# refresh-bio/colord

Measured on AMD Instinct MI355X. Metric: input Gbases/s + archive size vs ref, ONT 50 Gb at 1/2/4/8 MI355X, higher is better.
Workload: dtype u64

## Files before the change

colord_amd/_native.py:

```python
from __future__ import annotations
import ctypes as C
import os

os.environ.setdefault("GPU_MAX_HW_QUEUES", "32")
_HERE = os.path.dirname(os.path.abspath(__file__))
LIB_PATH = os.environ.get("COLORD_HIP_LIBRARY") or os.path.join(_HERE, "libcolord_hip.so")

CL_OK, CL_E_INVALID, CL_E_HIP, CL_E_CAPACITY, CL_E_NOMEM, CL_E_UNSUPPORTED, CL_E_MISMATCH = 0, -1, -2, -3, -4, -5, -6


class ColordHipError(RuntimeError):
    def __init__(self, status, msg):
        super().__init__(f"colord_hip error {status}: {msg}")
        self.status = status


class QualParams(C.Structure):
    _fields_ = [("mode", C.c_int32), ("source", C.c_int32), ("level", C.c_int32), ("n_fwd", C.c_uint32), ("fwd", C.c_uint32 * 8),
                ("n_rev", C.c_uint32), ("rev", C.c_uint32 * 8)]


class KmerStats(C.Structure):
    _fields_ = [("n_reads", C.c_uint64), ("tot_kmers", C.c_uint64), ("n_unique", C.c_uint64),
                ("n_unique_counted", C.c_uint64), ("total_count_filtered", C.c_uint64)]
# ... 128 lines not shown
    "cl_accepted_kmers": (C.c_int32, [_P, _P, _P, C.c_uint32, C.c_uint32, C.POINTER(_P)]),
    "cl_kmer_lists_free": (None, [_P]),
    "cl_kmer_lists_reads": (C.c_uint32, [_P]),
    "cl_kmer_lists_total": (C.c_uint64, [_P]),
    "cl_kmer_lists_offsets": (_P, [_P]),
    "cl_kmer_lists_kmers": (_P, [_P]),
    "cl_kmer_lists_ids": (_P, [_P]),
    "cl_kmer_lists_pos": (_P, [_P]),
    "cl_ref_accept": (C.c_int32, [C.c_uint32, C.c_uint32, C.c_uint32, C.c_double, _P]),
    "cl_index_build": (C.c_int32, [_P, _P, _P, _P, C.c_uint32, C.c_uint32, C.POINTER(_P)]),
    "cl_index_entries_of": (C.c_int32, [_P, _P, _P, C.c_uint32, _P, _P, C.c_uint64, C.POINTER(C.c_uint64), _P, C.POINTER(C.c_uint32)]),
    "cl_index_build_pairs": (C.c_int32, [_P, _P, _P, _P, C.c_uint64, _P, C.c_uint32, C.c_uint32, C.c_uint32, C.c_uint32, C.POINTER(_P)]),
    "cl_index_free": (None, [_P]),
    "cl_index_n_refs": (C.c_uint32, [_P]),
    "cl_index_entries": (C.c_uint64, [_P]),
    "cl_index_ref_rank": (_P, [_P]),
    "cl_candidates": (C.c_int32, [_P, _P, _P, C.c_uint32, _P, _P, _P]),
    "cl_candidates_common": (C.c_int32, [_P, _P, _P, C.c_uint32, _P, _P, _P, _P, C.c_uint64, C.POINTER(C.c_uint64)]),
    "cl_qual_coder_create": (C.c_int32, [_P, C.POINTER(QualParams), C.POINTER(_P)]),
    "cl_qual_coder_ctx": (_P, [_P]),
    "cl_qual_coder_free": (None, [_P]),
    "cl_qual_coder_set_domain_symbols": (C.c_int32, [_P, C.c_uint64]),
    "cl_qual_coder_domains": (C.c_int32, [_P, _P, C.c_uint64, C.POINTER(C.c_uint64)]),
    "cl_qual_coder_model": (C.c_int32, [_P, C.c_uint32, C.c_uint64, _P, C.c_uint32, C.POINTER(C.c_uint32)]),
    "cl_qual_coder_groups": (C.c_int32, [_P, C.POINTER(C.c_uint64)]),
    "cl_compressor_set_qual_domain_symbols": (C.c_int32, [_P, C.c_uint64]),
    "cl_compressor_qual_domains": (C.c_int32, [_P, _P, C.c_uint64, C.POINTER(C.c_uint64)]),
    "cl_qual_decode_domains": (C.c_int32, [_P, C.POINTER(QualParams), _P, _P, _P, C.c_uint64, _P, _P, C.c_uint32, _P, C.c_uint32, C.c_uint32, _P, _P, C.c_uint64, _P, C.c_uint64]),
    "cl_qual_encode": (C.c_int32, [_P, _P, _P, _P, _P, _P, _P, C.c_uint32, _P, C.c_uint64, _P, C.POINTER(C.c_uint64)]),
    "cl_anchor_candidates": (C.c_int32, [_P, _P, _P, _P, _P, C.c_uint32, C.c_uint32, C.c_double, C.c_double, C.c_double, C.c_uint32, C.POINTER(_P)]),
    "cl_anchor_candidates_hifi": (C.c_int32, [_P, _P, _P, _P, _P, C.c_uint32, C.c_uint32, C.c_double, C.c_double, C.c_double, C.c_uint32, C.c_uint32, C.c_uint32, _P, _P, C.POINTER(_P)]),
    "cl_anchors_free": (None, [_P]),
    "cl_anchors_total": (C.c_uint64, [_P]),
    "cl_anchors_n_cands": (_P, [_P]),
    "cl_anchors_cands": (_P, [_P]),
    "cl_anchors_cand_offsets": (_P, [_P]),
    "cl_anchors_data": (_P, [_P]),
    "cl_encode_plain": (C.c_int32, [_P, _P, _P, C.c_uint64, _P, _P, C.POINTER(C.c_uint64)]),
    "cl_reads_select": (C.c_int32, [_P, _P, _P, C.POINTER(_P)]),
    "cl_reads_from_arena": (C.c_int32, [_P, _P, _P, _P, C.c_uint32, C.POINTER(_P)]),
    "cl_estimator_logs": (C.c_int32, [_P, _P, _P, C.c_uint64, _P]),
    "cl_es_flags": (C.c_int32, [_P, _P, _P, _P, _P, _P]),
    "cl_id_coder_create": (C.c_int32, [C.c_int32, C.POINTER(_P)]),
    "cl_id_coder_free": (None, [_P]),
    "cl_id_coder_error": (C.c_char_p, [_P]),
    "cl_id_encode_part": (C.c_int32, [_P, _P, _P, _P, C.c_uint32, _P, C.c_uint64, C.POINTER(C.c_uint64)]),
    "cl_compress_shard": (C.c_int32, [_P, C.POINTER(CompressParams), _P, _P, _P, _P, C.c_uint32, _P, C.c_uint32, _P, _P, _P, C.c_uint64, _P, _P, C.c_uint64, _P,
                                      C.POINTER(CompressInfo)]),
    "cl_candidates_at": (C.c_int32, [_P, _P, _P, _P, C.c_uint32, _P, _P, _P]),
    "cl_compressor_create": (C.c_int32, [_P, _P, C.POINTER(CompressParams), C.POINTER(QualParams), C.POINTER(Exchange), C.c_uint64, C.POINTER(_P)]),
    "cl_compressor_free": (None, [_P]),
    "cl_compressor_count_add": (C.c_int32, [_P, _P]),
    "cl_compressor_count_finish": (C.c_int32, [_P, C.POINTER(KmerStats)]),
    "cl_compressor_refs_add": (C.c_int32, [_P, _P]),
    "cl_compressor_refs_finish": (C.c_int32, [_P]),
    "cl_compressor_encode": (C.c_int32, [_P, _P, _P, _P, _P, C.c_uint32, _P, C.c_uint32, _P, C.c_uint64, _P, _P, C.c_uint64, _P, C.POINTER(CompressInfo)]),
    "cl_compressor_genome_add": (C.c_int32, [_P, _P]),
    "cl_compressor_pseudo_reads": (C.c_int32, [_P, _P]),
    "cl_genome_encode": (C.c_int32, [_P, _P, C.c_uint32, _P, C.c_uint64, C.POINTER(C.c_uint64)]),
    "cl_genome_decode": (C.c_int32, [_P, C.c_uint64, C.c_uint32, _P, C.c_uint64, _P, C.POINTER(C.c_uint64)]),
    "cl_genome_md5": (C.c_int32, [_P, _P, C.c_uint32, _P]),
    "cl_compressor_prepare": (C.c_int32, [_P, _P, _P, C.c_uint32]),
    "cl_compressor_prepare_parts": (C.c_int32, [_P, _P, _P, C.c_uint32, _P, C.c_uint32, _P, _P]),
    "cl_compressor_info": (C.c_int32, [_P, C.POINTER(KmerStats), C.POINTER(C.c_uint64), C.POINTER(C.c_uint64), C.POINTER(C.c_uint64), C.POINTER(C.c_uint32), C.POINTER(C.c_uint32)]),
    "cl_dna_decoder_create": (C.c_int32, [C.c_uint32, C.c_int32, C.c_uint32, C.c_uint32, C.c_int32, C.c_uint32, C.c_double, C.POINTER(_P)]),
    "cl_dna_decoder_free": (None, [_P]),
# ... 48 lines not shown
```

colord_amd/csrc/anchors.hip:

```cpp
#include "common.hpp"
#include "objects.hpp"
#include <algorithm>

struct cl_anchors {
	cl_ctx* ctx = nullptr;
	uint32_t n_reads = 0, c = 0;
	uint64_t n_anchors = 0;
	DevBuf<uint32_t> n_cands;
	DevBuf<uint32_t> cand;
	DevBuf<uint64_t> cand_off;
	DevBuf<uint32_t> anchors;
};

namespace {

struct Arena { const uint64_t* packed; const uint64_t* word_off; const uint32_t* lens; };

__device__ inline uint64_t mmer_at(const Arena& A, uint64_t wb, uint32_t p, uint32_t m)
{
	const uint64_t* w = A.packed + wb + (p >> 5);
	const uint32_t j = p & 31;
	const uint64_t hi = w[0], lo = w[1];
	const uint32_t s = 128 - 2 * (j + m);
	const uint64_t v = (s >= 64) ? (hi >> (s - 64)) : ((hi << (64 - s)) | (lo >> s));
	return v & ((1ULL << (2 * m)) - 1);
}
__device__ inline uint64_t mmer_of(uint64_t hi, uint64_t lo, uint32_t p, uint32_t m)
{
	const uint32_t s = 128 - 2 * ((p & 31) + m);
	const uint64_t v = (s >= 64) ? (hi >> (s - 64)) : ((hi << (64 - s)) | (lo >> s));
	return v & ((1ULL << (2 * m)) - 1);
}
__device__ inline uint64_t revcomp_m(uint64_t x, uint32_t m)
{
	x = ~x; x = __brevll(x);
	x = ((x >> 1) & 0x5555555555555555ULL) | ((x & 0x5555555555555555ULL) << 1);
	return x >> (64 - 2 * m);
}
__device__ inline uint64_t ref_mmer(const Arena& R, uint32_t id, bool rev, uint32_t q, uint32_t m)
{
	const uint32_t len = R.lens[id];
	const uint64_t wb = R.word_off[id];
	return rev ? revcomp_m(mmer_at(R, wb, len - m - q, m), m) : mmer_at(R, wb, q, m);
}
// ... 370 lines not shown
			};
			if (fill + tot > LSTAGE) flush();
			if (tot <= LSTAGE) { put(stage, (uint64_t)(fill + incl - cnt)); fill += tot; continue; }
			unsigned long long base = 0;
			if (lane == 0) base = atomicAdd(n_pairs, (unsigned long long)tot);
			base = ((unsigned long long)__shfl((int)(base >> 32), 0, 64) << 32) | (uint32_t)__shfl((int)(uint32_t)base, 0, 64);
			if (base + tot > cap) continue;
			put(pairs, (uint64_t)(base + incl - cnt));
		}
	}
	flush();
}
__global__ void k_task_pairs(const uint64_t* __restrict__ pairs, uint64_t n_pairs, Arena A, TaskCfg cfg, const uint32_t* __restrict__ n_distinct, uint32_t n_tasks,
                             uint64_t* __restrict__ pair_off, uint32_t* __restrict__ pair_cnt)
{
	const uint32_t t = blockIdx.x * blockDim.x + threadIdx.x;
	if (t > n_tasks) return;
	auto lower = [&](uint64_t task) -> uint64_t {
		const uint64_t key = task << (cfg.pe + cfg.pr);
		uint64_t lo = 0, hi = n_pairs;
		while (lo < hi) { const uint64_t mid = (lo + hi) >> 1; if (pairs[mid] < key) lo = mid + 1; else hi = mid; }
		return lo;
	};
	const uint64_t a = lower(t);
	pair_off[t] = a;
	if (t == n_tasks) return;
	uint32_t total = (uint32_t)(lower((uint64_t)t + 1) - a);
	const uint32_t rl = t / (2 * cfg.c); const uint32_t elen = A.lens[cfg.r0 + rl];
	const bool always = (double)n_distinct[rl] > cfg.frac_always * (double)elen;
	if (!always && (double)total > cfg.max_mult * (double)(elen + 1)) total = 0;
	pair_cnt[t] = total;
}

__device__ inline int lis_search(const int* __restrict__ tf, int size, int value)
{
	int low = 0;
	while (size > 0)
	{
		const int half = size / 2, other_half = size - half, probe = low + half, other_low = low + other_half;
		const int v = tf[probe];
		size = half;
		low = value > v ? other_low : low;
	}
	return low;
}
__global__ __launch_bounds__(64) void k_lis_anchors(Arena A, Arena R, TaskCfg cfg, const uint32_t* __restrict__ cand_refs, uint32_t n_tasks,
                                                   const uint64_t* __restrict__ pair_off, const uint32_t* __restrict__ pair_cnt, const uint64_t* __restrict__ pairs,
                                                   int* __restrict__ tf, int* __restrict__ ts, int* __restrict__ pred,
                                                   uint32_t* __restrict__ anch, uint32_t* __restrict__ t_nanch, uint32_t* __restrict__ t_tot, uint32_t dbg)
{
	__builtin_amdgcn_s_setprio(3);
	const uint32_t t = blockIdx.x * blockDim.x + threadIdx.x;
	if (t >= n_tasks) return;
	const uint64_t a = pair_off[t], b = a + pair_cnt[t];
	uint32_t n_anch = 0, tot = 0;
	if (b > a)
	{
		const uint32_t n = (uint32_t)(b - a);
		const uint64_t* P = pairs + a;
		int* F = tf + a; int* S = ts + a; int* PR = pred + a;
		const uint32_t pr_mask = (1u << cfg.pr) - 1, pe_mask = (1u << cfg.pe) - 1;
		auto ref_pos = [&](uint32_t i) -> int { return (int)(~(uint32_t)P[i] & pr_mask); };
		auto enc_pos = [&](uint32_t i) -> uint32_t { return (uint32_t)(P[i] >> cfg.pr) & pe_mask; };
		F[0] = ref_pos(0); S[0] = 0; PR[0] = -1;
		int out_len = 1;
		int last_f = F[0], last_s = 0;
		for (int i = 1; i < (int)n; ++i)
		{
			const int x = ref_pos((uint32_t)i);
			if (last_f < x)
			{
				F[out_len] = x; S[out_len] = i; PR[i] = last_s;
				++out_len; last_f = x; last_s = i;
				continue;
			}
			const int pos = lis_search(F, out_len, x);
			F[pos] = x; S[pos] = i;
			PR[i] = pos > 0 ? S[pos - 1] : -1;
			if (pos == out_len - 1) { last_f = x; last_s = i; }
		}
		if (dbg == 1) { t_nanch[t] = 0; t_tot[t] = 0; return; }
		int cur = S[out_len - 1];
		for (int i = out_len - 1; i >= 0; --i) { F[i] = cur; cur = PR[cur]; }
		if (dbg == 2) { t_nanch[t] = 0; t_tot[t] = 0; return; }
		const uint32_t rl = t / (2 * cfg.c), slot = (t / 2) % cfg.c; const bool rev = (t & 1) == 0;
		const uint32_t r = cfg.r0 + rl;
		const uint32_t id = cand_refs[(uint64_t)r * cfg.c + slot];
// ... 21 lines not shown
		int idx3 = idx_of(2);
		uint64_t pw2 = P[idx_of(1)];
		Raw w1 = words_of(P[idx_of(0)]);
		for (int i = 0; i < out_len; ++i)
		{
			const uint32_t pr = w1.pr, e_own = w1.e;
			const uint64_t mraw = m_from(w1.r0, w1.r1, w1.rp), mm = rev ? revcomp_m(mraw, cfg.m) : mraw, am = m_from(w1.a0, w1.a1, w1.e);
			w1 = words_of(pw2);
			pw2 = P[idx3];
			idx3 = idx_of(i + 3);
			uint32_t pe;
			for (;;)
			{
				pe = pe_at_ep;
				const bool hit = (pe == e_own ? am : mmer_at(A, ewb, pe, cfg.m)) == mm;
				uint32_t nxt = pe;
				do { ++ep; nxt = pe_ahead; pe_ahead = ep + 1 < n ? enc_pos(ep + 1) : 0xffffffffu; } while (ep < n && nxt == pe);
				pe_at_ep = nxt;
				if (hit || ep >= n) break;
			}
			if (run && prev_e == pe - 1 && prev_r == pr - 1) ++run;
			else
			{
				if (run) { out[3 * n_anch] = run + cfg.m - 1; out[3 * n_anch + 1] = start_e; out[3 * n_anch + 2] = start_r; tot += run + cfg.m - 1; ++n_anch; }
				run = 1; start_e = pe; start_r = pr;
			}
			prev_e = pe; prev_r = pr;
		}
		if (run) { out[3 * n_anch] = run + cfg.m - 1; out[3 * n_anch + 1] = start_e; out[3 * n_anch + 2] = start_r; tot += run + cfg.m - 1; ++n_anch; }
	}
	t_nanch[t] = n_anch; t_tot[t] = tot;
}

struct KmerArgs {
	const uint64_t* common; const uint64_t* common_off;
	uint64_t* sorted; uint32_t* tab;
	uint32_t* kanch;
	uint32_t* k_n; uint32_t* k_tot; uint8_t* k_use;
	uint64_t base;
	uint32_t k; ModTest mt;
};
__device__ inline uint32_t oriented_sym(const Arena& R, uint64_t wb, uint32_t len, bool rev, uint32_t pos)
{
	const uint32_t p = rev ? len - 1 - pos : pos;
	const uint32_t b = (uint32_t)(R.packed[wb + (p >> 5)] >> (62 - 2 * (p & 31))) & 3u;
	return rev ? 3u - b : b;
}
__device__ inline void kmer_occurrences(const Arena& A, uint64_t wb, uint32_t len, uint32_t k, const ModTest& mt, const uint64_t* sorted, uint32_t n, uint32_t* cntF, uint32_t* posF, uint32_t* cntR, uint32_t* posR)
{
	for (uint32_t i = 0; i < n; ++i) { cntF[i] = cntR[i] = 0; posF[i] = posR[i] = 0; }
	if (len < k) return;
	const uint64_t mask = (1ULL << (2 * k)) - 1; uint64_t f = 0, r = 0;
	for (uint32_t p = 0; p < len; ++p)
	{
		const uint64_t b = (A.packed[wb + (p >> 5)] >> (62 - 2 * (p & 31))) & 3u;
		f = ((f << 2) + b) & mask; r = (r >> 2) + ((3 - b) << (2 * (k - 1)));
		if (p + 1 < k) continue;
		const uint64_t can = f < r ? f : r;
		if (!mod_is_zero(hash_mm(can), mt)) continue;
		uint32_t lo = 0, hi = n;
		while (lo < hi) { const uint32_t mid = (lo + hi) >> 1; if (sorted[mid] < can) lo = mid + 1; else hi = mid; }
		if (lo >= n || sorted[lo] != can) continue;
		if (f == can) { ++cntF[lo]; posF[lo] = p + 1 - k; } else { ++cntR[lo]; posR[lo] = p + 1 - k; }
	}
}
__device__ inline uint32_t kmer_anchor_chain(const Arena& A, uint64_t ewb, uint32_t elen, const Arena& R, uint64_t rwb, uint32_t rlen, bool rev, uint32_t k,
// ... 199 lines not shown
	HIP_TRY(ctx, hipSetDevice(ctx->device));
	const uint32_t nr = reads->n_reads, m = anchor_len;
	cl_anchors* X = new cl_anchors(); X->ctx = ctx; X->n_reads = nr; X->c = c;
	std::unique_ptr<cl_anchors> guard(X);
	DEV_ALLOC(ctx, X->n_cands, nr); DEV_ALLOC(ctx, X->cand, (uint64_t)nr * c * 4); DEV_ALLOC(ctx, X->cand_off, (uint64_t)nr * c + 1);
	Arena A{ reads->packed.p, reads->word_off.p, reads->lens.p }, R{ refs->packed.p, refs->word_off.p, refs->lens.p };
	std::vector<uint32_t> h_len(nr);
	if (nr) HIP_TRY(ctx, hipMemcpy(h_len.data(), reads->lens.p, (uint64_t)nr * 4, hipMemcpyDeviceToHost));
	auto bits_for = [](uint64_t v) -> uint32_t { uint32_t b = 1; while ((1ull << b) <= v) ++b; return b; };
	uint32_t max_ref_len = 0;
	if (refs->n_reads)
	{
		std::vector<uint32_t> rl(refs->n_reads);
		HIP_TRY(ctx, hipMemcpy(rl.data(), refs->lens.p, (uint64_t)refs->n_reads * 4, hipMemcpyDeviceToHost));
		for (uint32_t l : rl) max_ref_len = std::max(max_ref_len, l);
	}
	const uint32_t pr_bits = bits_for(max_ref_len);
	const uint64_t BATCH_BASES = 1ull << 28;
	std::vector<DevBuf<uint32_t>> chunks; std::vector<uint64_t> chunk_n;
	uint64_t total_anchors = 0;
	double pairs_per_base = 0.5;
	struct TableBatch {
		uint32_t r0 = 0, r1 = 0, pe = 1; uint64_t acc = 0, nsum = 0;
		DevBuf<uint32_t> n_distinct, next, err; DevBuf<uint64_t> toff, noff; DevBuf<EncSlot> slots; DevBuf<uint2> bins;
		std::vector<uint2> h_work; DevBuf<uint2> work;
		struct SideSync { hipStream_t s = nullptr; ~SideSync() { if (s) (void)hipStreamSynchronize(s); } } sync;
	};
	HIP_TRY(ctx, cl_side_stream(ctx, ctx->side));
	constexpr uint32_t LDS_N_A = 12288, LDS_N_B = 24576, LDS_NT = 1024;
	uint32_t lds_max_n = 0;
	if (const char* e = getenv("COLORD_HIP_ANCHORS_LDS")) lds_max_n = atoi(e) <= 0 ? 0u : (uint32_t)atoi(e) <= LDS_N_A ? LDS_N_A : LDS_N_B;
	const uint32_t match_seg = getenv("COLORD_HIP_MATCH_SEG") ? (uint32_t)std::max(0, atoi(getenv("COLORD_HIP_MATCH_SEG"))) : 16384u;
	const uint32_t lds_dbg = getenv("COLORD_HIP_LDS_DBG") ? (uint32_t)atoi(getenv("COLORD_HIP_LDS_DBG")) : 0u;
	auto prepare = [&](uint32_t r0, std::unique_ptr<TableBatch>& out) -> cl_status {
		out = std::make_unique<TableBatch>();
		TableBatch& B = *out;
		uint32_t r1 = r0; uint64_t acc = 0;
		uint32_t mx = 0;
		while (r1 < nr && (r1 == r0 || acc + h_len[r1] <= BATCH_BASES))
		{
			const uint32_t pe = bits_for(std::max(mx, h_len[r1]));
			if (r1 > r0 && pe + pr_bits + bits_for((r1 - r0 + 1) * 2 * c) > 64) break;
			mx = std::max(mx, h_len[r1]); acc += h_len[r1]; ++r1;
		}
		B.r0 = r0; B.r1 = r1; B.acc = acc; B.pe = bits_for(mx);
		for (uint32_t r = r0; r < r1; ++r)
			for (uint32_t sg = 0, ns = match_segments(h_len[r] >= m ? h_len[r] - m + 1 : 0, match_seg); sg < ns; ++sg) B.h_work.push_back(make_uint2(r - r0, sg));
		if (B.pe + pr_bits + bits_for((r1 - r0) * 2 * c) > 64) return cl_fail(ctx, CL_E_UNSUPPORTED, "cl_anchor_candidates: a read and its candidates are too long for 64-bit match keys");
		const uint32_t nb = r1 - r0;
		const uint32_t table_x4 = 8;
		LaunchOn on(ctx, ctx->side);
		B.sync.s = ctx->side;
		DevBuf<uint32_t> tsize, nsize, err; DEV_ALLOC(ctx, tsize, nb); DEV_ALLOC(ctx, nsize, nb); DEV_ALLOC(ctx, err, 1); DEV_ALLOC(ctx, B.n_distinct, nb);
		HIP_TRY(ctx, hipMemsetAsync(err.p, 0, 4, ctx->side));
		LAUNCH(ctx, k_table_sizes, grid_for(nb, 256), 256, (const uint32_t*)reads->lens.p, (const uint8_t*)reads->has_n.p, d_cand_n, r0, r1, m, table_x4, lds_max_n, tsize.p, nsize.p, err.p);
		DEV_ALLOC(ctx, B.toff, (uint64_t)nb + 1); DEV_ALLOC(ctx, B.noff, (uint64_t)nb + 1);
		uint64_t tsum = 0;
		CL_TRY(dev_exclusive_scan_u64(ctx, tsize.p, B.toff.p, nb, &tsum));
		CL_TRY(dev_exclusive_scan_u64(ctx, nsize.p, B.noff.p, nb, &B.nsum));
		uint32_t herr = 0; HIP_TRY(ctx, hipMemcpyAsync(&herr, err.p, 4, hipMemcpyDeviceToHost, ctx->side)); HIP_TRY(ctx, hipStreamSynchronize(ctx->side));
		DEV_ALLOC(ctx, B.slots, tsum); DEV_ALLOC(ctx, B.next, B.nsum); DEV_ALLOC(ctx, B.bins, B.nsum); DEV_ALLOC(ctx, B.err, 1);
		DEV_ALLOC(ctx, B.work, B.h_work.size() + 1);
		if (!B.h_work.empty()) HIP_TRY(ctx, hipMemcpyAsync(B.work.p, B.h_work.data(), B.h_work.size() * sizeof(uint2), hipMemcpyHostToDevice, ctx->side));
		HIP_TRY(ctx, hipMemsetAsync(B.n_distinct.p, 0, (uint64_t)nb * 4, ctx->side));
		HIP_TRY(ctx, hipMemsetAsync(B.err.p, 0, 4, ctx->side));
		EncTable T{ B.slots.p, B.toff.p, B.next.p, B.noff.p };
// ... 24 lines not shown
			DEV_ALLOC(ctx, pairs, cap);
			HIP_TRY(ctx, hipMemsetAsync(d_np.p, 0, 32, ctx->stream));
			if (lds_max_n)
			{
				LAUNCH_NAMED(ctx, "k_match_lds<12288>", (k_match_lds<LDS_N_A, 2048, LDS_NT, 8>), nb, LDS_NT, A, R, cfg, 0u, (const uint8_t*)reads->has_n.p, d_cand_refs, d_cand_n, n_distinct.p, nb, d_np.p, cap, pairs.p, lds_dbg);
				if (lds_max_n > LDS_N_A)
					LAUNCH_NAMED(ctx, "k_match_lds<24576>", (k_match_lds<LDS_N_B, 4096, LDS_NT, 4>), nb, LDS_NT, A, R, cfg, LDS_N_A, (const uint8_t*)reads->has_n.p, d_cand_refs, d_cand_n, n_distinct.p, nb, d_np.p, cap, pairs.p, lds_dbg);
			}
			LAUNCHB(ctx, 0.0, k_match, (uint32_t)cur->h_work.size(), 256, A, R, T, cfg, d_cand_refs, d_cand_n, (const uint32_t*)n_distinct.p, (const uint2*)cur->work.p, (uint32_t)cur->h_work.size(), match_seg, d_np.p, cap, pairs.p);
			HIP_TRY(ctx, hipGetLastError());
			unsigned long long h_np2[2] = { 0, 0 };
			HIP_TRY(ctx, hipMemcpyAsync(h_np2, d_np.p, 16, hipMemcpyDeviceToHost, ctx->stream));
			if (r1 < nr && !nxt) CL_TRY(prepare(r1, nxt));
			HIP_TRY(ctx, hipStreamSynchronize(ctx->stream));
			const unsigned long long h_np = h_np2[0];
			n_pairs = h_np;
			if (ctx->timing && !ctx->pending_bytes.empty()) ctx->pending_bytes.back() = (double)h_np2[1] * 8.25 + (double)std::min<uint64_t>(h_np, cap) * 8.0;
			if (getenv("COLORD_HIP_ANCHOR_DEBUG")) fprintf(stderr, "[anchors] batch reads %u..%u bases %llu: pairs %llu cap %llu\n", r0, r1, (unsigned long long)acc, h_np, (unsigned long long)cap);
			if (n_pairs >= (1ull << 32)) return cl_fail(ctx, CL_E_UNSUPPORTED, "cl_anchor_candidates: batch produces >= 2^32 match pairs");
			if (n_pairs <= cap) break;
			cap = n_pairs;
		}
		if (acc) pairs_per_base = std::max(pairs_per_base, (double)n_pairs / (double)acc);
		DevBuf<int> tf, ts, pred; DEV_ALLOC(ctx, tf, n_pairs); DEV_ALLOC(ctx, ts, n_pairs); DEV_ALLOC(ctx, pred, n_pairs);
		DevBuf<uint32_t> anch; DEV_ALLOC(ctx, anch, 3 * n_pairs);
		DevBuf<uint32_t> t_nanch, t_tot; DEV_ALLOC(ctx, t_nanch, n_tasks); DEV_ALLOC(ctx, t_tot, n_tasks);
		if (n_pairs)
		{
			uint32_t tb = 1; while ((1ull << tb) < n_tasks) ++tb;
			CL_TRY(dev_sort_pairs(ctx, pairs.p, nullptr, n_pairs, 0, cfg.pe + cfg.pr + tb));
		}
		LAUNCH(ctx, k_task_pairs, grid_for((uint64_t)n_tasks + 1, 256), 256, (const uint64_t*)pairs.p, n_pairs, A, cfg, (const uint32_t*)n_distinct.p, n_tasks, pair_off.p, pair_cnt.p);
		LAUNCHB(ctx, n_pairs * 32.0, k_lis_anchors, grid_for(n_tasks, 64), 64, A, R, cfg, d_cand_refs, n_tasks, (const uint64_t*)pair_off.p, (const uint32_t*)pair_cnt.p, (const uint64_t*)pairs.p,
			tf.p, ts.p, pred.p, anch.p, t_nanch.p, t_tot.p, (uint32_t)(getenv("COLORD_HIP_LIS_DBG") ? atoi(getenv("COLORD_HIP_LIS_DBG")) : 0));
		HIP_TRY(ctx, hipGetLastError());
		const uint64_t n_slots = (uint64_t)nb * c;
		DevBuf<uint64_t> k_sorted; DevBuf<uint32_t> k_tab, kanch, k_n, k_tot; DevBuf<uint8_t> k_use;
		uint64_t common_base = 0;
		if (hifi)
		{
			uint64_t hb[2] = { 0, 0 };
			HIP_TRY(ctx, hipMemcpy(&hb[0], d_common_off + (uint64_t)r0 * c, 8, hipMemcpyDeviceToHost));
			HIP_TRY(ctx, hipMemcpy(&hb[1], d_common_off + (uint64_t)r1 * c, 8, hipMemcpyDeviceToHost));
			common_base = hb[0];
			const uint64_t nk = hb[1] - hb[0];
			DEV_ALLOC(ctx, k_sorted, nk + 1); DEV_ALLOC(ctx, k_tab, 8 * nk + 8); DEV_ALLOC(ctx, kanch, 6 * nk + 6);
			DEV_ALLOC(ctx, k_n, 2 * n_slots); DEV_ALLOC(ctx, k_tot, 2 * n_slots); DEV_ALLOC(ctx, k_use, n_slots);
			KmerArgs ka{ d_common, d_common_off, k_sorted.p, k_tab.p, kanch.p, k_n.p, k_tot.p, k_use.p, common_base, kmer_len, make_modtest(modulo) };
			LAUNCH(ctx, k_kmer_anchors, grid_for(n_slots, 64), 64, A, R, cfg, d_cand_refs, d_cand_n, (const uint8_t*)reads->has_n.p, (const uint32_t*)n_distinct.p, ka);
			HIP_TRY(ctx, hipGetLastError());
		}
		DevBuf<uint32_t> o_task, o_count; DEV_ALLOC(ctx, o_task, n_slots); DEV_ALLOC(ctx, o_count, n_slots);
		LAUNCH(ctx, k_select, grid_for(nb, 128), 128, cfg, d_cand_refs, d_cand_n, min_anchors, (const uint32_t*)t_nanch.p, (const uint32_t*)t_tot.p,
			(const uint8_t*)(hifi ? k_use.p : nullptr), (const uint32_t*)k_n.p, (const uint32_t*)k_tot.p,
			X->n_cands.p, X->cand.p, o_task.p, o_count.p);
		DevBuf<uint64_t> slot_off; DEV_ALLOC(ctx, slot_off, n_slots + 1);
		uint64_t n_here = 0;
		CL_TRY(dev_exclusive_scan_u64(ctx, o_count.p, slot_off.p, n_slots, &n_here));
		DevBuf<uint32_t> chunk; DEV_ALLOC(ctx, chunk, 3 * n_here);
		LAUNCH(ctx, k_copy_fix, grid_for(n_slots, 128), 128, (const uint32_t*)o_task.p, (const uint64_t*)slot_off.p, n_slots, (const uint64_t*)pair_off.p,
			(const uint32_t*)anch.p, (uint64_t)0, chunk.p, cfg, (const uint32_t*)kanch.p, d_common_off, common_base);
		HIP_TRY(ctx, hipMemcpyAsync(X->cand_off.p + (uint64_t)r0 * c, slot_off.p, n_slots * 8, hipMemcpyDeviceToDevice, ctx->stream));
		if (total_anchors) LAUNCH(ctx, k_add_u64, grid_for(n_slots, 256), 256, X->cand_off.p + (uint64_t)r0 * c, n_slots, total_anchors);
		HIP_TRY(ctx, hipGetLastError());
		HIP_TRY(ctx, hipStreamSynchronize(ctx->stream));
		chunks.push_back(std::move(chunk)); chunk_n.push_back(n_here);
		total_anchors += n_here;
		cur = std::move(nxt);
	}
	X->n_anchors = total_anchors;
	DEV_ALLOC(ctx, X->anchors, 3 * total_anchors);
	uint64_t o = 0;
	for (size_t i = 0; i < chunks.size(); ++i)
	{
		if (chunk_n[i]) HIP_TRY(ctx, hipMemcpyAsync(X->anchors.p + 3 * o, chunks[i].p, chunk_n[i] * 12, hipMemcpyDeviceToDevice, ctx->stream));
		o += chunk_n[i];
	}
	HIP_TRY(ctx, hipMemcpyAsync(X->cand_off.p + (uint64_t)nr * c, &total_anchors, 8, hipMemcpyHostToDevice, ctx->stream));
	HIP_TRY(ctx, hipStreamSynchronize(ctx->stream));
	cl_timing_collect(ctx);
	*out = guard.release();
	return CL_OK;
}
extern "C" void cl_anchors_free(cl_anchors* a) { delete a; }
extern "C" uint64_t cl_anchors_total(const cl_anchors* a) { return a->n_anchors; }
extern "C" const uint32_t* cl_anchors_n_cands(const cl_anchors* a) { return a->n_cands.p; }
extern "C" const uint32_t* cl_anchors_cands(const cl_anchors* a) { return a->cand.p; }
extern "C" const uint64_t* cl_anchors_cand_offsets(const cl_anchors* a) { return a->cand_off.p; }
extern "C" const uint32_t* cl_anchors_data(const cl_anchors* a) { return a->anchors.p; }
```

colord_amd/device.py:

```python
from __future__ import annotations
import ctypes as C
import numpy as np
import torch
from . import _native as N


def _check(ctx, st):
    if ctx is not None and getattr(ctx, "timing", False):
        for n, (ms, k, b, cells) in ctx.kernel_times().items():
            a = ctx.acc.setdefault(n, [0.0, 0, 0.0, 0.0])
            a[0] += ms
            a[1] += k
            a[2] += b
            a[3] += cells
    if st != N.CL_OK:
        msg = N.load().cl_last_error(ctx.h).decode() if ctx is not None and ctx.h else ""
        raise N.ColordHipError(st, msg)


def _view(ptr, n, dtype, device):
    out = torch.empty(int(n), dtype=dtype, device=device)
    if n:
        torch.cuda.synchronize(device)
        rc = _hip().hipMemcpy(C.c_void_p(out.data_ptr()), C.c_void_p(ptr), C.c_size_t(int(n) * out.element_size()), 3)
# ... 757 lines not shown
    def __init__(self, ctx, h, max_alt_refs):
        super().__init__(ctx, h)
        self.max_alt_refs = max_alt_refs

    def encode(self, refs: "Reads", es: torch.Tensor, es_off: torch.Tensor, es_ntuples: torch.Tensor, part_bounds):
        ctx = self.ctx
        pb = np.ascontiguousarray(part_bounds, dtype=np.uint32)
        n_parts = len(pb) - 1
        n_reads = es_off.numel() - 1
        sizes = np.zeros(max(n_parts, 1), np.uint64)
        cap = max(4096, int(es.numel() * 0.6) + 64 * n_parts)
        out = torch.empty(cap, dtype=torch.uint8, device=ctx.device)
        n = C.c_uint64(0)
        st = ctx.lib.cl_dna_encode(ctx.h, self.h, refs.h, es.data_ptr(), es_off.data_ptr(), es_ntuples.data_ptr(), n_reads,
                                   pb.ctypes.data, n_parts, out.data_ptr(), cap, sizes.ctypes.data, C.byref(n))
        _check(ctx, st)
        return out[:n.value], [int(x) for x in sizes[:n_parts]]

    def model(self, family: int, context: int) -> np.ndarray:
        out = np.zeros(257, np.uint32)
        _check(self.ctx, self.ctx.lib.cl_dna_coder_model(self.h, family, context, out.ctypes.data))
        return out[:(self.N_SYM[family] or self.max_alt_refs) + 1].copy()


class Anchors(_Obj):
    _free = "cl_anchors_free"

    def __init__(self, ctx, h, n_reads, c):
        super().__init__(ctx, h)
        self.n_reads, self.c = n_reads, c

    @property
    def total(self): return self.ctx.lib.cl_anchors_total(self.h)
    def n_cands(self): return self._arr("cl_anchors_n_cands", self.n_reads, torch.int32)
    def cands(self): return self._arr("cl_anchors_cands", self.n_reads * self.c * 4, torch.int32).view(self.n_reads, self.c, 4)
    def cand_offsets(self): return self._arr("cl_anchors_cand_offsets", self.n_reads * self.c + 1, torch.int64)
    def data(self): return self._arr("cl_anchors_data", self.total * 3, torch.int32).view(-1, 3)
```

include/colord_hip.h:

```cpp
#ifndef COLORD_HIP_H
#define COLORD_HIP_H
#include <stdint.h>
#include <stddef.h>

#ifdef __cplusplus
extern "C" {
#endif

typedef int32_t cl_status;
enum {
	CL_OK = 0,
	CL_E_INVALID = -1,
	CL_E_HIP = -2,
	CL_E_CAPACITY = -3,
	CL_E_NOMEM = -4,
	CL_E_UNSUPPORTED = -5,
	CL_E_MISMATCH = -6
};

typedef struct cl_ctx cl_ctx;
typedef struct cl_reads cl_reads;
typedef struct cl_kmer_set cl_kmer_set;
typedef struct cl_kmer_lists cl_kmer_lists;
typedef struct cl_index cl_index;
// ... 81 lines not shown

typedef struct cl_qual_coder cl_qual_coder;
typedef struct {
	int32_t mode;
	int32_t source;
	int32_t level;
	uint32_t n_fwd;
	uint32_t fwd[8];
	uint32_t n_rev;
	uint32_t rev[8];
} cl_qual_params;
cl_status cl_qual_coder_create(cl_ctx* ctx, const cl_qual_params* params, cl_qual_coder** out);
void cl_qual_coder_free(cl_qual_coder* q);
cl_ctx* cl_qual_coder_ctx(const cl_qual_coder* q);
cl_status cl_qual_encode(cl_ctx* ctx, cl_qual_coder* q, const cl_reads* reads, const uint8_t* d_quals, const uint64_t* d_qual_off,
                         const uint8_t* d_flags, const uint32_t* h_part_bounds, uint32_t n_parts,
                         uint8_t* d_out, uint64_t cap, uint64_t* h_part_sizes, uint64_t* n_out);

cl_status cl_qual_coder_set_domain_symbols(cl_qual_coder* q, uint64_t n);
cl_status cl_qual_coder_domains(const cl_qual_coder* q, uint64_t* h_first_part, uint64_t cap, uint64_t* n_out);
cl_status cl_qual_coder_model(const cl_qual_coder* q, uint32_t family, uint64_t context, uint32_t* out, uint32_t cap, uint32_t* n_out);
cl_status cl_qual_coder_groups(const cl_qual_coder* q, uint64_t* n_out);

typedef struct cl_anchors cl_anchors;
cl_status cl_anchor_candidates(cl_ctx* ctx, const cl_reads* reads, const cl_reads* refs, const uint32_t* d_cand_refs, const uint32_t* d_cand_n,
                               uint32_t c, uint32_t anchor_len, double frac_always, double frac_min, double max_matches_mult,
                               uint32_t min_anchors, cl_anchors** out);
cl_status cl_anchor_candidates_hifi(cl_ctx* ctx, const cl_reads* reads, const cl_reads* refs, const uint32_t* d_cand_refs, const uint32_t* d_cand_n,
                                    uint32_t c, uint32_t anchor_len, double frac_always, double frac_min, double max_matches_mult,
                                    uint32_t min_anchors, uint32_t kmer_len, uint32_t modulo, const uint64_t* d_common_off, const uint64_t* d_common,
                                    cl_anchors** out);
void cl_anchors_free(cl_anchors* a);
uint64_t cl_anchors_total(const cl_anchors* a);
const uint32_t* cl_anchors_n_cands(const cl_anchors* a);
const uint32_t* cl_anchors_cands(const cl_anchors* a);
const uint64_t* cl_anchors_cand_offsets(const cl_anchors* a);
const uint32_t* cl_anchors_data(const cl_anchors* a);

cl_status cl_encode_plain(cl_ctx* ctx, const cl_reads* reads, uint8_t* d_es, uint64_t cap, uint64_t* d_es_off,
                          uint32_t* d_es_ntuples, uint64_t* n_out);

cl_status cl_encode_reads(cl_ctx* ctx, const cl_reads* reads, const cl_reads* refs, const cl_anchors* anchors, uint32_t c, uint32_t anchor_len,
                          uint32_t min_part_alt, uint32_t max_rec, double cost_mult, const uint32_t* h_pack_bounds, uint32_t n_packs,
                          uint8_t* d_es, uint64_t cap, uint64_t* d_es_off, uint32_t* d_es_ntuples, uint64_t* n_out);

cl_status cl_estimator_logs(cl_ctx* ctx, const uint32_t* d_count, const uint32_t* d_total, uint64_t n, double* d_out);

cl_status cl_es_flags(cl_ctx* ctx, const cl_reads* reads, const uint8_t* d_es, const uint64_t* d_es_off, const uint64_t* d_base_off, uint8_t* d_flags);

cl_status cl_es_expand(cl_ctx* ctx, const cl_reads* refs, const uint8_t* d_es, const uint64_t* d_es_off, const uint32_t* d_es_ntuples, uint32_t n_reads,
                       uint8_t* d_codes, uint64_t cap, uint64_t* d_base_off, uint64_t* n_out);
cl_status cl_es_verify(cl_ctx* ctx, const cl_reads* reads, const cl_reads* refs, const uint8_t* d_es, const uint64_t* d_es_off, const uint32_t* d_es_ntuples,
                       uint64_t* n_bad, uint32_t* first_bad);

cl_status cl_digest_bases(cl_ctx* ctx, const cl_reads* reads, uint64_t first_read, cl_digest* acc);
cl_status cl_digest_quals(cl_ctx* ctx, const cl_qual_params* qparams, const cl_reads* reads, const uint8_t* d_quals, const uint64_t* d_qual_off,
                          uint64_t first_read, cl_digest* acc);
cl_status cl_digest_bases_host(const uint8_t* h_codes, const uint64_t* h_off, uint64_t n, uint64_t first_read, cl_digest* acc);
cl_status cl_digest_bytes_host(uint32_t kind, const uint8_t* h_bytes, const uint64_t* h_off, uint64_t n, uint64_t first_read, cl_digest* acc);
cl_status cl_digest_qual_values(cl_ctx* ctx, const cl_qual_params* qparams, const cl_reads* reads, const uint8_t* d_quals, const uint64_t* d_qual_off,
                                uint64_t first_read, cl_digest* acc);
cl_status cl_qual_values(cl_ctx* ctx, const cl_qual_params* qparams, const cl_reads* reads, const uint8_t* d_quals, const uint64_t* d_qual_off,
                         uint8_t* d_values, uint64_t cap);
cl_status cl_qual_values_host(const cl_qual_params* qparams, const uint8_t* h_quals, const uint64_t* h_off, uint64_t n, uint8_t* h_values);
cl_status cl_digest_qual_values_host(const uint8_t* h_ascii_quals, const uint64_t* h_off, uint64_t n, uint64_t first_read, cl_digest* acc);

// ... 154 lines not shown
```

Measured before the change: 2.927.

## Chain long anchor candidate lists with a whole wavefront instead of one lane

Tasks whose pair list has at least a threshold number of entries (default 64) are skipped by the per-lane LIS kernel. A new kernel then processes each such task with a full 64-lane wavefront: it extends runs with ballots, uses a wave-parallel binary search for the LIS, backtracks in parallel and emits anchors cooperatively. The aim is to remove load imbalance and serial latency from lanes stuck on long lists. It adds an extra kernel launch, atomic counters with a reduction kernel and a small device-to-host copy, and brings complex lane-cooperative logic that must match the serial output exactly.

```diff
diff --git a/colord_amd/_native.py b/colord_amd/_native.py
--- a/colord_amd/_native.py
+++ b/colord_amd/_native.py
@@ -184,6 +184,10 @@
     "cl_anchor_candidates_hifi": (C.c_int32, [_P, _P, _P, _P, _P, C.c_uint32, C.c_uint32, C.c_double, C.c_double, C.c_double, C.c_uint32, C.c_uint32, C.c_uint32, _P, _P, C.POINTER(_P)]),
     "cl_anchors_free": (None, [_P]),
     "cl_anchors_total": (C.c_uint64, [_P]),
+    "cl_anchors_wave_tasks": (C.c_uint64, [_P]),
+    "cl_anchors_wave_pairs": (C.c_uint64, [_P]),
+    "cl_anchors_lane_tasks": (C.c_uint64, [_P]),
+    "cl_anchors_lane_pairs": (C.c_uint64, [_P]),
     "cl_anchors_n_cands": (_P, [_P]),
     "cl_anchors_cands": (_P, [_P]),
     "cl_anchors_cand_offsets": (_P, [_P]),
diff --git a/colord_amd/csrc/anchors.hip b/colord_amd/csrc/anchors.hip
--- a/colord_amd/csrc/anchors.hip
+++ b/colord_amd/csrc/anchors.hip
@@ -10,6 +10,8 @@
 	DevBuf<uint32_t> cand;
 	DevBuf<uint64_t> cand_off;
 	DevBuf<uint32_t> anchors;
+	DevBuf<unsigned long long> lis_counts_d;
+	unsigned long long lis_counts[6] = { 0, 0, 0, 0, 0, 0 };
 };
 
 namespace {
@@ -446,6 +448,22 @@
 	pair_cnt[t] = total;
 }
 
+constexpr uint32_t LIS_COUNT_LINES = 1024;
+__device__ inline unsigned long long shfl_xor_u64(unsigned long long v, int d)
+{
+	return ((unsigned long long)(uint32_t)__shfl_xor((int)(v >> 32), d, 64) << 32) | (uint32_t)__shfl_xor((int)(uint32_t)v, d, 64);
+}
+__global__ __launch_bounds__(64) void k_lis_counts_sum(unsigned long long* __restrict__ counts)
+{
+	unsigned long long v[6] = { 0, 0, 0, 0, 0, 0 };
+	for (uint32_t l = threadIdx.x; l < LIS_COUNT_LINES; l += 64)
+		for (int k = 0; k < 6; ++k) { const unsigned long long x = counts[(size_t)l * 8 + k]; v[k] = k == 5 ? max(v[k], x) : v[k] + x; }
+	for (int d = 32; d; d >>= 1)
+		for (int k = 0; k < 6; ++k) { const unsigned long long x = shfl_xor_u64(v[k], d); v[k] = k == 5 ? max(v[k], x) : v[k] + x; }
+	__syncthreads();
+	if (threadIdx.x == 0) for (int k = 0; k < 6; ++k) counts[k] = v[k];
+}
+
 __device__ inline int lis_search(const int* __restrict__ tf, int size, int value)
 {
 	int low = 0;
@@ -461,12 +479,25 @@
 __global__ __launch_bounds__(64) void k_lis_anchors(Arena A, Arena R, TaskCfg cfg, const uint32_t* __restrict__ cand_refs, uint32_t n_tasks,
                                                    const uint64_t* __restrict__ pair_off, const uint32_t* __restrict__ pair_cnt, const uint64_t* __restrict__ pairs,
                                                    int* __restrict__ tf, int* __restrict__ ts, int* __restrict__ pred,
-                                                   uint32_t* __restrict__ anch, uint32_t* __restrict__ t_nanch, uint32_t* __restrict__ t_tot, uint32_t dbg)
+                                                   uint32_t* __restrict__ anch, uint32_t* __restrict__ t_nanch, uint32_t* __restrict__ t_tot,
+                                                   uint32_t wave_min, unsigned long long* __restrict__ counts, uint32_t dbg)
 {
 	__builtin_amdgcn_s_setprio(3);
 	const uint32_t t = blockIdx.x * blockDim.x + threadIdx.x;
-	if (t >= n_tasks) return;
-	const uint64_t a = pair_off[t], b = a + pair_cnt[t];
+	const uint32_t n_own = t < n_tasks ? pair_cnt[t] : 0;
+	const bool others = n_own && wave_min && n_own >= wave_min;
+	{
+		unsigned long long sum = others ? 0 : n_own; uint32_t mx = (uint32_t)sum;
+		for (int d = 32; d; d >>= 1) { sum += shfl_xor_u64(sum, d); mx = max(mx, (uint32_t)__shfl_xor((int)mx, d, 64)); }
+		const uint32_t tasks = (uint32_t)__popcll(__ballot(n_own && !others));
+		if ((threadIdx.x & 63) == 0 && tasks)
+		{
+			unsigned long long* cl = counts + (size_t)(blockIdx.x % LIS_COUNT_LINES) * 8;
+			atomicAdd(cl + 2, (unsigned long long)tasks); atomicAdd(cl + 3, sum); atomicMax(cl + 5, (unsigned long long)mx);
+		}
+	}
+	if (t >= n_tasks || others) return;
+	const uint64_t a = pair_off[t], b = a + n_own;
 	uint32_t n_anch = 0, tot = 0;
 	if (b > a)
 	{
@@ -554,6 +585,182 @@
 	t_nanch[t] = n_anch; t_tot[t] = tot;
 }
 
+__device__ inline void lis_wave_fence() { __builtin_amdgcn_fence(__ATOMIC_ACQ_REL, "workgroup"); }
+__device__ inline uint64_t shfl_u64(uint64_t v, uint32_t src)
+{
+	return ((uint64_t)(uint32_t)__shfl((int)(v >> 32), (int)src, 64) << 32) | (uint32_t)__shfl((int)(uint32_t)v, (int)src, 64);
+}
+__device__ inline uint32_t ones_from_bit0(uint64_t b) { return b == ~0ULL ? 64u : (uint32_t)__builtin_ctzll(~b); }
+__device__ inline int lis_search_wave(const int* F, int size, int value, uint32_t lane)
+{
+	int lo = 0;
+	while (size > 0)
+	{
+		const int piece = (size + 63) >> 6, end = lo + size;
+		const long long idx = (long long)lo + ((long long)lane + 1) * piece - 1;
+		const bool less = idx < end && F[idx] < value;
+		lo += __popcll(__ballot(less)) * piece;
+		size = min(piece - 1, end - lo);
+	}
+	return lo;
+}
+constexpr uint32_t LIS_WAVE_GAP = 8;
+constexpr uint32_t LIS_WAVE_BLOCK = 256;
+constexpr uint32_t LIS_WAVE_MIN_DEFAULT = 64;
+__global__ __launch_bounds__(LIS_WAVE_BLOCK) void k_lis_anchors_wave(Arena A, Arena R, TaskCfg cfg, const uint32_t* __restrict__ cand_refs, uint32_t n_tasks,
+                                                        const uint64_t* __restrict__ pair_off, const uint32_t* __restrict__ pair_cnt, const uint64_t* __restrict__ pairs,
+                                                        int* tf, int* ts, int* pred, uint32_t* __restrict__ anch, uint32_t* __restrict__ t_nanch, uint32_t* __restrict__ t_tot,
+                                                        uint32_t wave_min, unsigned long long* __restrict__ counts, uint32_t dbg)
+{
+	__builtin_amdgcn_s_setprio(3);
+	const uint32_t lane = threadIdx.x & 63;
+	const uint32_t t = __builtin_amdgcn_readfirstlane(blockIdx.x * (LIS_WAVE_BLOCK / 64) + (threadIdx.x >> 6));
+	if (t >= n_tasks) return;
+	const uint32_t n = pair_cnt[t];
+	if (n == 0 || n < wave_min) return;
+	const uint64_t a = pair_off[t];
+	const uint64_t* P = pairs + a;
+	int* F = tf + a; int* S = ts + a; int* PR = pred + a;
+	const uint32_t m = cfg.m, pr_mask = (1u << cfg.pr) - 1, pe_mask = (1u << cfg.pe) - 1;
+	auto ref_pos = [&](uint32_t i) -> int { return (int)(~(uint32_t)P[i] & pr_mask); };
+	auto enc_pos = [&](uint32_t i) -> uint32_t { return (uint32_t)(P[i] >> cfg.pr) & pe_mask; };
+	unsigned long long* cl = counts + (size_t)(blockIdx.x % LIS_COUNT_LINES) * 8;
+	if (lane == 0) { atomicAdd(cl, 1ULL); atomicAdd(cl + 1, (unsigned long long)n); atomicMax(cl + 5, (unsigned long long)n); }
+	uint32_t n_slow = 0;
+	int out_len = 0, last_f = -1, last_s = -1;
+	for (uint32_t i0 = 0; i0 < n; i0 += 64)
+	{
+		const uint32_t cnt = min(64u, n - i0);
+		const int x = lane < cnt ? ref_pos(i0 + lane) : 0;
+		const int xp = __shfl_up(x, 1, 64);
+		uint32_t k0 = 0;
+		while (k0 < cnt)
+		{
+			const bool ext = lane >= k0 && lane < cnt && x > (lane == k0 ? last_f : xp);
+			const uint32_t r = ones_from_bit0(__ballot(ext) >> k0);
+			if (r)
+			{
+				if (lane >= k0 && lane < k0 + r)
+				{
+					F[out_len + (int)(lane - k0)] = x; S[out_len + (int)(lane - k0)] = (int)(i0 + lane);
+					PR[i0 + lane] = lane == k0 ? last_s : (int)(i0 + lane) - 1;
+				}
+				out_len += (int)r; k0 += r;
+				last_f = __shfl(x, (int)k0 - 1, 64); last_s = (int)(i0 + k0) - 1;
+			}
+			if (k0 < cnt)
+			{
+				const int xs = __shfl(x, (int)k0, 64);
+				lis_wave_fence();
+				const int pos = lis_search_wave(F, out_len, xs, lane);
+				const int before = pos > 0 ? S[pos - 1] : -1;
+				if (lane == 0) { F[pos] = xs; S[pos] = (int)(i0 + k0); PR[i0 + k0] = before; }
+				if (pos == out_len - 1) { last_f = xs; last_s = (int)(i0 + k0); }
+				++k0; ++n_slow;
+			}
+		}
+	}
+	if (lane == 0 && n_slow) atomicAdd(cl + 4, (unsigned long long)n_slow);
+	if (dbg == 1) { if (lane == 0) { t_nanch[t] = 0; t_tot[t] = 0; } return; }
+	lis_wave_fence();
+	{
+		int cur = S[out_len - 1];
+		for (int i = out_len - 1; i >= 0; )
+		{
+			const int nv = min(64, i + 1);
+			const bool in = (int)lane < nv && cur - (int)lane >= 0;
+			const int pv = in ? PR[cur - (int)lane] : -2;
+			const int run = (int)ones_from_bit0(__ballot(in && pv == cur - (int)lane - 1));
+			const int last = min(run, nv - 1);
+			if ((int)lane <= last) F[i - (int)lane] = cur - (int)lane;
+			cur = __shfl(pv, last, 64);
+			i -= last + 1;
+		}
+	}
+	if (dbg == 2) { if (lane == 0) { t_nanch[t] = 0; t_tot[t] = 0; } return; }
+	lis_wave_fence();
+	const uint32_t rl = t / (2 * cfg.c), slot = (t / 2) % cfg.c; const bool rev = (t & 1) == 0;
+	const uint32_t r = cfg.r0 + rl;
+	const uint32_t id = cand_refs[(uint64_t)r * cfg.c + slot];
+	const uint64_t ewb = A.word_off[r];
+	const uint32_t rlen = R.lens[id]; const uint64_t rwb = R.word_off[id];
+	uint32_t* out = anch + 3 * a;
+	uint32_t from = 0, skip = 0xffffffffu;
+	uint32_t run = 0, start_e = 0, start_r = 0, prev_e = 0, prev_r = 0, n_anch = 0;
+	for (uint32_t i = 0; i < (uint32_t)out_len; )
+	{
+		const uint32_t cnt = min(64u, (uint32_t)out_len - i);
+		const bool valid = lane < cnt;
+		uint32_t idx = 0, pe = 0, pr = 0; uint64_t mm = 0;
+		if (valid)
+		{
+			idx = (uint32_t)F[i + lane];
+			const uint64_t pw = P[idx];
+			pr = ~(uint32_t)pw & pr_mask; pe = (uint32_t)(pw >> cfg.pr) & pe_mask;
+			const uint64_t mraw = mmer_at(R, rwb, rev ? rlen - m - pr : pr, m);
+			mm = rev ? revcomp_m(mraw, m) : mraw;
+		}
+		const uint32_t idx_b = (uint32_t)__shfl_up((int)idx, 1, 64), pe_b = (uint32_t)__shfl_up((int)pe, 1, 64);
+		const uint32_t st = lane == 0 ? from : idx_b + 1, sk = lane == 0 ? skip : pe_b;
+		bool fail = false;
+		if (valid)
+		{
+			fail = idx < st || idx - st > LIS_WAVE_GAP || mmer_at(A, ewb, pe, m) != mm;
+			for (uint32_t j = st; !fail && j < idx; ++j)
+			{
+				const uint32_t ej = enc_pos(j);
+				fail = ej != sk && ej != pe && mmer_at(A, ewb, ej, m) == mm;
+			}
+		}
+		const uint64_t fb = __ballot(valid && fail);
+		const uint32_t f = fb ? (uint32_t)__builtin_ctzll(fb) : cnt;
+		uint32_t g = f;
+		if (f < cnt)
+		{
+			const uint64_t mmf = shfl_u64(mm, f);
+			const uint32_t stf = (uint32_t)__shfl((int)st, (int)f, 64), skf = (uint32_t)__shfl((int)sk, (int)f, 64);
+			uint32_t q = 0, jq = 0; bool found = false;
+			for (uint32_t j0 = stf; j0 < n && !found; j0 += 64)
+			{
+				const uint32_t j = j0 + lane; uint32_t ej = 0; bool hit = false;
+				if (j < n) { ej = enc_pos(j); hit = ej != skf && mmer_at(A, ewb, ej, m) == mmf; }
+				const uint64_t hb = __ballot(hit);
+				if (hb) { const int hl = __builtin_ctzll(hb); q = (uint32_t)__shfl((int)ej, hl, 64); jq = j0 + (uint32_t)hl; found = true; }
+			}
+			if (!found) { q = enc_pos(n - 1); jq = n - 1; }
+			if (lane == f) pe = q;
+			g = f + 1; from = jq + 1; skip = q;
+		}
+		else { from = (uint32_t)__shfl((int)idx, (int)cnt - 1, 64) + 1; skip = (uint32_t)__shfl((int)pe, (int)cnt - 1, 64); }
+		const uint32_t pe_p = (uint32_t)__shfl_up((int)pe, 1, 64), pr_p = (uint32_t)__shfl_up((int)pr, 1, 64);
+		const bool goes_on = lane == 0 ? (run && prev_e == pe - 1 && prev_r == pr - 1) : (pe_p == pe - 1 && pr_p == pr - 1);
+		const bool head = lane < g && !goes_on;
+		const uint64_t hb = __ballot(head);
+		if (hb)
+		{
+			const uint32_t h0 = (uint32_t)__builtin_ctzll(hb), hl = 63u - (uint32_t)__builtin_clzll(hb);
+			const uint32_t base = n_anch + (run ? 1u : 0u);
+			if (run && lane == 0) { out[3 * n_anch] = run + h0 + m - 1; out[3 * n_anch + 1] = start_e; out[3 * n_anch + 2] = start_r; }
+			const uint64_t later = hb & ~((2ULL << lane) - 1);
+			if (head && later)
+			{
+				const uint32_t w = base + (uint32_t)__popcll(hb & ((1ULL << lane) - 1));
+				out[3 * w] = (uint32_t)__builtin_ctzll(later) - lane + m - 1; out[3 * w + 1] = pe; out[3 * w + 2] = pr;
+			}
+			n_anch = base + (uint32_t)__popcll(hb) - 1;
+			run = g - hl; start_e = (uint32_t)__shfl((int)pe, (int)hl, 64); start_r = (uint32_t)__shfl((int)pr, (int)hl, 64);
+		}
+		else run += g;
+		prev_e = (uint32_t)__shfl((int)pe, (int)g - 1, 64); prev_r = (uint32_t)__shfl((int)pr, (int)g - 1, 64);
+		i += g;
+	}
+	if (lane == 0)
+	{
+		if (run) { out[3 * n_anch] = run + m - 1; out[3 * n_anch + 1] = start_e; out[3 * n_anch + 2] = start_r; ++n_anch; }
+		t_nanch[t] = n_anch; t_tot[t] = (uint32_t)out_len + n_anch * (m - 1);
+	}
+}
+
 struct KmerArgs {
 	const uint64_t* common; const uint64_t* common_off;
 	uint64_t* sorted; uint32_t* tab;
@@ -819,6 +1026,10 @@
 	if (const char* e = getenv("COLORD_HIP_ANCHORS_LDS")) lds_max_n = atoi(e) <= 0 ? 0u : (uint32_t)atoi(e) <= LDS_N_A ? LDS_N_A : LDS_N_B;
 	const uint32_t match_seg = getenv("COLORD_HIP_MATCH_SEG") ? (uint32_t)std::max(0, atoi(getenv("COLORD_HIP_MATCH_SEG"))) : 16384u;
 	const uint32_t lds_dbg = getenv("COLORD_HIP_LDS_DBG") ? (uint32_t)atoi(getenv("COLORD_HIP_LDS_DBG")) : 0u;
+	const uint32_t lis_wave_min = getenv("COLORD_HIP_LIS_WAVE_MIN") ? (uint32_t)std::max(0, atoi(getenv("COLORD_HIP_LIS_WAVE_MIN"))) : LIS_WAVE_MIN_DEFAULT;
+	const uint32_t lis_dbg = getenv("COLORD_HIP_LIS_DBG") ? (uint32_t)atoi(getenv("COLORD_HIP_LIS_DBG")) : 0u;
+	DEV_ALLOC(ctx, X->lis_counts_d, (uint64_t)LIS_COUNT_LINES * 8);
+	HIP_TRY(ctx, hipMemsetAsync(X->lis_counts_d.p, 0, (uint64_t)LIS_COUNT_LINES * 64, ctx->stream));
 	auto prepare = [&](uint32_t r0, std::unique_ptr<TableBatch>& out) -> cl_status {
 		out = std::make_unique<TableBatch>();
 		TableBatch& B = *out;
@@ -909,7 +1120,10 @@
 		}
 		LAUNCH(ctx, k_task_pairs, grid_for((uint64_t)n_tasks + 1, 256), 256, (const uint64_t*)pairs.p, n_pairs, A, cfg, (const uint32_t*)n_distinct.p, n_tasks, pair_off.p, pair_cnt.p);
 		LAUNCHB(ctx, n_pairs * 32.0, k_lis_anchors, grid_for(n_tasks, 64), 64, A, R, cfg, d_cand_refs, n_tasks, (const uint64_t*)pair_off.p, (const uint32_t*)pair_cnt.p, (const uint64_t*)pairs.p,
-			tf.p, ts.p, pred.p, anch.p, t_nanch.p, t_tot.p, (uint32_t)(getenv("COLORD_HIP_LIS_DBG") ? atoi(getenv("COLORD_HIP_LIS_DBG")) : 0));
+			tf.p, ts.p, pred.p, anch.p, t_nanch.p, t_tot.p, lis_wave_min, X->lis_counts_d.p, lis_dbg);
+		if (lis_wave_min)
+			LAUNCH(ctx, k_lis_anchors_wave, grid_for(n_tasks, LIS_WAVE_BLOCK / 64), LIS_WAVE_BLOCK, A, R, cfg, d_cand_refs, n_tasks, (const uint64_t*)pair_off.p, (const uint32_t*)pair_cnt.p, (const uint64_t*)pairs.p,
+				tf.p, ts.p, pred.p, anch.p, t_nanch.p, t_tot.p, lis_wave_min, X->lis_counts_d.p, lis_dbg);
 		HIP_TRY(ctx, hipGetLastError());
 		const uint64_t n_slots = (uint64_t)nb * c;
 		DevBuf<uint64_t> k_sorted; DevBuf<uint32_t> k_tab, kanch, k_n, k_tot; DevBuf<uint8_t> k_use;
@@ -954,13 +1168,22 @@
 		o += chunk_n[i];
 	}
 	HIP_TRY(ctx, hipMemcpyAsync(X->cand_off.p + (uint64_t)nr * c, &total_anchors, 8, hipMemcpyHostToDevice, ctx->stream));
+	LAUNCH(ctx, k_lis_counts_sum, 1, 64, X->lis_counts_d.p);
+	HIP_TRY(ctx, hipMemcpyAsync(X->lis_counts, X->lis_counts_d.p, 48, hipMemcpyDeviceToHost, ctx->stream));
 	HIP_TRY(ctx, hipStreamSynchronize(ctx->stream));
+	if (getenv("COLORD_HIP_ANCHOR_DEBUG"))
+		fprintf(stderr, "[anchors] chained by a wave: %llu tasks %llu pairs (%llu did not extend); by a lane: %llu tasks %llu pairs; longest list %llu; threshold %u\n",
+			X->lis_counts[0], X->lis_counts[1], X->lis_counts[4], X->lis_counts[2], X->lis_counts[3], X->lis_counts[5], lis_wave_min);
 	cl_timing_collect(ctx);
 	*out = guard.release();
 	return CL_OK;
 }
 extern "C" void cl_anchors_free(cl_anchors* a) { delete a; }
 extern "C" uint64_t cl_anchors_total(const cl_anchors* a) { return a->n_anchors; }
+extern "C" uint64_t cl_anchors_wave_tasks(const cl_anchors* a) { return a->lis_counts[0]; }
+extern "C" uint64_t cl_anchors_wave_pairs(const cl_anchors* a) { return a->lis_counts[1]; }
+extern "C" uint64_t cl_anchors_lane_tasks(const cl_anchors* a) { return a->lis_counts[2]; }
+extern "C" uint64_t cl_anchors_lane_pairs(const cl_anchors* a) { return a->lis_counts[3]; }
 extern "C" const uint32_t* cl_anchors_n_cands(const cl_anchors* a) { return a->n_cands.p; }
 extern "C" const uint32_t* cl_anchors_cands(const cl_anchors* a) { return a->cand.p; }
 extern "C" const uint64_t* cl_anchors_cand_offsets(const cl_anchors* a) { return a->cand_off.p; }
diff --git a/colord_amd/device.py b/colord_amd/device.py
--- a/colord_amd/device.py
+++ b/colord_amd/device.py
@@ -813,6 +813,11 @@
 
     @property
     def total(self): return self.ctx.lib.cl_anchors_total(self.h)
+
+    def lis_counts(self):
+        lib = self.ctx.lib
+        return ((lib.cl_anchors_wave_tasks(self.h), lib.cl_anchors_wave_pairs(self.h)), (lib.cl_anchors_lane_tasks(self.h), lib.cl_anchors_lane_pairs(self.h)))
+
     def n_cands(self): return self._arr("cl_anchors_n_cands", self.n_reads, torch.int32)
     def cands(self): return self._arr("cl_anchors_cands", self.n_reads * self.c * 4, torch.int32).view(self.n_reads, self.c, 4)
     def cand_offsets(self): return self._arr("cl_anchors_cand_offsets", self.n_reads * self.c + 1, torch.int64)
diff --git a/include/colord_hip.h b/include/colord_hip.h
--- a/include/colord_hip.h
+++ b/include/colord_hip.h
@@ -137,6 +137,10 @@
                                     cl_anchors** out);
 void cl_anchors_free(cl_anchors* a);
 uint64_t cl_anchors_total(const cl_anchors* a);
+uint64_t cl_anchors_wave_tasks(const cl_anchors* a);
+uint64_t cl_anchors_wave_pairs(const cl_anchors* a);
+uint64_t cl_anchors_lane_tasks(const cl_anchors* a);
+uint64_t cl_anchors_lane_pairs(const cl_anchors* a);
 const uint32_t* cl_anchors_n_cands(const cl_anchors* a);
 const uint32_t* cl_anchors_cands(const cl_anchors* a);
 const uint64_t* cl_anchors_cand_offsets(const cl_anchors* a);
```

Result: faster. 3.084, median of 6 (+5.4%).
